# FishYuLi/BalancedGroupSoftmax

Measured on AMD Instinct MI355X. Metric: img/s fwd+bwd R50-FPN+BAGS 1333x800, 512 RoI (BASELINE metric: img/s/GPU fwd+bwd R50-FPN+BAGS 1333x800, 512 RoI; GroupSoftmax us/RoI), higher is better.
Workload: dtype f32 (conv/linear products on the bf16 MFMA from exact 3-way bf16 splits, fp32 accumulate: fp32-faithful)

## Files before the change

balancedgroupsoftmax_amd/backbone.py:

```python
import contextlib

import torch
import torch.nn as nn

from . import functional as BF
from .ops import OFFSET_PITCH, DeformConv
from .registry import BACKBONES, NECKS


def _trainable(*modules):
    return torch.is_grad_enabled() and any(
        p.requires_grad for m in modules if m is not None for p in m.parameters())


def _fold_conv_bn(conv, bn, pad_cin_to=None):
    w = conv.weight
    cbias = getattr(conv, 'bias', None)
    if w.is_cuda:
        ctx = contextlib.nullcontext() if _trainable(conv, bn) else torch.no_grad()
        with ctx:
            if bn is not None:
                return BF.fold_conv_bn(w, cbias, bn.weight, bn.bias, bn.running_mean,
                                       bn.running_var, bn.eps, cin_padded=pad_cin_to)
            return BF.fold_conv_bn(w, cbias, cin_padded=pad_cin_to)
# ... 148 lines not shown
        if self.groups > 1:
            out = BF.grouped_conv3x3_nhwc(out, f['c2'][0], f['c2'][1], self.groups, stride=self.stride,
                                          relu=True)
        else:
            out = BF.conv2d_nhwc(out, f['c2'][0], f['c2'][1], stride=self.stride, pad=1, relu=True)
        if fk is not None:
            fk.join()
        return BF.conv2d_nhwc(out, f['c3'][0], f['c3'][1], relu=True, residual=identity)

    def run(self, x, f, next_c1=None, h=None):
        if h is not None and (x.dtype == torch.bfloat16 or self.groups > 1 or self.with_dcn or
                              (torch.is_grad_enabled() and x.requires_grad)):
            raise RuntimeError('Bottleneck.run: a precomputed conv1 output is for the frozen fp32 block only')
        if x.dtype == torch.bfloat16:
            return self.run_bf16_storage(x, f)
        tagged = bool(getattr(x, '_bgs_consumers_mask', False))
        fuse = BF.fork_fusion_enabled() and torch.is_grad_enabled() and x.requires_grad
        if tagged and not fuse:
            raise RuntimeError("Bottleneck.run: x is a relu='consumers' block output but fork fusion is off")
        out_relu = 'consumers' if BF.fork_fusion_enabled() else True
        xin = x
        identity = x
        fk = None
        if 'ds' in f and not fuse and x.is_cuda and BF.shortcut_fork_enabled() and \
                not (torch.is_grad_enabled() and any(t.requires_grad for t in f['ds'] if t is not None)):
            with BF.forked(x.device) as fk:
                identity = BF.conv2d_nhwc(x, f['ds'][0], f['ds'][1], stride=self.stride)
        elif 'ds' in f:
            if fuse:
                identity, xin = BF.conv2d_autograd(x, f['ds'][0], f['ds'][1], stride=self.stride,
                                                   mask_input=tagged, passthrough=True)
            else:
                identity = BF.conv2d_autograd(x, f['ds'][0], f['ds'][1], stride=self.stride)
        first_pt = fuse and 'ds' not in f
        first_mask = tagged and 'ds' not in f
        if self.groups > 1 or self.with_dcn:
            out = BF.conv2d_autograd(xin, f['c1'][0], f['c1'][1], relu=True, mask_input=first_mask,
                                     passthrough=first_pt)
            if first_pt:
                out, identity = out
            if self.with_dcn:
                off = BF.conv2d_autograd(out, f['off'][0], f['off'][1], stride=self.stride, pad=1)
                out = BF.deform_conv3x3_nhwc(out, off, f['c2'][0], f['c2'][1], self.dcn_groups,
                                             stride=self.stride, relu=True)
            else:
                out = BF.grouped_conv3x3_nhwc(out, f['c2'][0], f['c2'][1], self.groups,
                                              stride=self.stride, relu=True)
            if fk is not None:
                fk.join()
            return BF.conv2d_autograd(out, f['c3'][0], f['c3'][1], relu=out_relu, residual=identity)
        if h is not None:
            out = h
        else:
            out = BF.conv2d_autograd(xin, f['c1'][0], f['c1'][1], relu='consumers', mask_input=first_mask,
                                     passthrough=first_pt)
            if first_pt:
                out, identity = out
        if not fuse and BF.fused_c3_eligible(out, f['c2'][0], f['c3'][0], self.stride, identity):
            if fk is not None:
                fk.join()
            if next_c1 is not None and BF.fused_c3_next_eligible(out, f['c2'][0], f['c3'][0], self.stride, identity,
                                                                 next_c1[0], next_c1[1]):
                return BF.conv3x3_c3_next_fused_nhwc(out, f['c2'][0], f['c2'][1], f['c3'][0], f['c3'][1], next_c1[0],
                                                     next_c1[1], residual=identity, relu3=True)
            return BF.conv3x3_c3_fused_nhwc(out, f['c2'][0], f['c2'][1], f['c3'][0], f['c3'][1], residual=identity,
                                            relu3=True)
        out = BF.conv2d_autograd(out, f['c2'][0], f['c2'][1], stride=self.stride, pad=1,
                                 relu='consumers', mask_input=True)
        if fk is not None:
            fk.join()
        return BF.conv2d_autograd(out, f['c3'][0], f['c3'][1], relu=out_relu, residual=identity,
                                  mask_input=True)


@BACKBONES.register_module
class ResNet(nn.Module):
    arch_settings = {50: (3, 4, 6, 3), 101: (3, 4, 23, 3), 152: (3, 8, 36, 3)}

    def __init__(self, depth, num_stages=4, strides=(1, 2, 2, 2), dilations=(1, 1, 1, 1),
                 out_indices=(0, 1, 2, 3), style='pytorch', frozen_stages=-1, conv_cfg=None,
# ... 217 lines not shown
```

balancedgroupsoftmax_amd/capi.py:

```python
import ctypes
import os

_PKG = os.path.dirname(os.path.abspath(__file__))

c_i64p = ctypes.c_void_p
c_f32p = ctypes.c_void_p
c_ptr = ctypes.c_void_p

BGS_OK = 0
BGS_MAX_BINS = 16


class BgsLibraryError(RuntimeError):
    pass


class BgsCallError(RuntimeError):
    def __init__(self, fn, code, text):
        super().__init__('%s failed with code %d: %s' % (fn, code, text))
        self.code = code


SIGNATURES = {
    'bgs_version': (ctypes.c_int, []),
# ... 56 lines not shown
                             + [c_f32p] * 4 + [c_ptr]),
    'bgs_conv2d_wgrad_bfx_workspace_bytes': (ctypes.c_size_t, [ctypes.c_int] * 9),
    'bgs_conv2d_wgrad_nhwc_f32_bfx': (ctypes.c_int, [c_f32p, c_f32p, c_f32p, c_f32p]
                                      + [ctypes.c_int] * 11 + [c_ptr, c_ptr]),
    'bgs_conv2d_wgrad_bfx_enable': (None, [ctypes.c_int]),
    'bgs_conv3x3_halo_nhwc_f32': (ctypes.c_int, [c_f32p, c_f32p, c_f32p, c_f32p] + [ctypes.c_int] * 6
                                  + [c_ptr]),
    'bgs_conv_bfx_weight_bytes': (ctypes.c_size_t, [ctypes.c_int, ctypes.c_int]),
    'bgs_conv_bfx_split_weights': (ctypes.c_int, [c_f32p, c_ptr, ctypes.c_int, ctypes.c_int, c_ptr]),
    'bgs_conv_dgrad_parity_enable': (None, [ctypes.c_int]),
    'bgs_conv_bfx_split_weights_dgrad': (ctypes.c_int, [c_f32p, c_ptr] + [ctypes.c_int] * 4 + [c_ptr]),
    'bgs_conv_bfx_workspace_bytes': (ctypes.c_size_t, [ctypes.c_longlong, ctypes.c_int, ctypes.c_int]),
    'bgs_conv2d_nhwc_f32_bfx_ws': (ctypes.c_int, [c_f32p, c_ptr, c_f32p, c_f32p, c_f32p]
                                   + [ctypes.c_int] * 12 + [c_ptr, ctypes.c_size_t, c_ptr]),
    'bgs_conv2d_dgrad_nhwc_f32_bfx_ws': (ctypes.c_int, [c_f32p, c_ptr, c_f32p, c_f32p, c_f32p]
                                         + [ctypes.c_int] * 11 + [c_ptr, ctypes.c_size_t, c_ptr]),
    'bgs_conv3x3_halo_bfx_workspace_bytes': (ctypes.c_size_t, [ctypes.c_int] * 5),
    'bgs_conv3x3_c3_fused_nhwc_f32_bfx': (ctypes.c_int, [c_f32p, c_ptr, c_f32p, c_ptr, c_f32p, c_f32p, c_f32p]
                                          + [ctypes.c_int] * 6 + [c_ptr]),
    'bgs_conv3x3_c3_next_fused_nhwc_f32_bfx': (ctypes.c_int,
                                               [c_f32p, c_ptr, c_f32p, c_ptr, c_f32p, c_f32p, c_f32p, c_ptr, c_f32p,
                                                c_f32p] + [ctypes.c_int] * 7 + [c_ptr]),
    'bgs_conv3x3_c3_next_eligible': (ctypes.c_int, [ctypes.c_int] * 6),
    'bgs_conv3x3_halo_nhwc_f32_bfx': (ctypes.c_int, [c_f32p, c_ptr, c_f32p, c_f32p]
                                      + [ctypes.c_int] * 7 + [c_ptr, ctypes.c_size_t, c_ptr]),
    'bgs_conv3x3_halo_nhwc_f32_bfx_ex': (ctypes.c_int, [c_f32p, c_ptr, c_f32p, c_f32p, c_f32p]
                                         + [ctypes.c_int] * 7 + [c_ptr, ctypes.c_size_t, c_ptr]),
    'bgs_conv3x3_planes_head_nhwc_f32_bfx': (ctypes.c_int, [c_f32p, c_ptr, c_f32p, c_ptr, c_f32p, c_f32p]
                                             + [ctypes.c_int] * 7 + [c_ptr]),
    'bgs_conv3x3_planes_head_eligible': (ctypes.c_int, [ctypes.c_int] * 6),
    'bgs_gs_loss_tuning': (None, [ctypes.c_int]),
    'bgs_gs_head_fold': (None, [ctypes.c_int]),
    'bgs_gs_loss_wavepriv_min_rows': (None, [ctypes.c_int]),
    'bgs_gs_merge_tuning': (None, [ctypes.c_int, ctypes.c_int]),
    'bgs_conv_bfx_wide_tuning': (None, [ctypes.c_int] * 3),
    'bgs_conv_bfx_wide_last_launch': (ctypes.c_int, []),
    'bgs_conv1x1_planes_enable': (None, [ctypes.c_int]),
    'bgs_conv1x1_planes_last_launch': (ctypes.c_int, []),
    'bgs_conv3x3_planes_enable': (None, [ctypes.c_int]),
    'bgs_conv3x3_planes_last_launch': (ctypes.c_int, []),
    'bgs_conv1x1_bres_enable': (None, [ctypes.c_int]),
    'bgs_conv1x1_bres_last_launch': (ctypes.c_int, []),
    'bgs_launch_census': (ctypes.c_int, [ctypes.c_int, ctypes.c_int]),
    'bgs_conv_bfx_tuning': (None, [ctypes.c_int] * 2),
    'bgs_conv_bfx_last_launch': (ctypes.c_int, [c_ptr, c_ptr]),
    'bgs_conv_tuning': (None, [ctypes.c_int] * 4),
# ... 235 lines not shown
```

balancedgroupsoftmax_amd/csrc/bottleneck_tail_planes.hip:

```cpp
#include <stdlib.h>

#include "conv_args.h"
#include "bfx_split.h"

using namespace bgs_conv;

namespace {

typedef __bf16 bf16x2 __attribute__((ext_vector_type(2)));
typedef __bf16 bf16x8 __attribute__((ext_vector_type(8)));
typedef unsigned u32x2 __attribute__((ext_vector_type(2)));
typedef unsigned u32x4 __attribute__((ext_vector_type(4)));

__device__ __forceinline__ unsigned pk_bf16(float a, float b) {
  const bf16x2 h = __builtin_convertvector(f32x2{a, b}, bf16x2);
  return __builtin_bit_cast(unsigned, h);
}

__device__ __forceinline__ void split3p(const f32x4 v, u32x2& hi, u32x2& mid, u32x2& lo) {
  hi = u32x2{pk_bf16(v[0], v[1]), pk_bf16(v[2], v[3])};
  const f32x4 r = {bfx_resid_lo(hi[0], v[0]), bfx_resid_hi(hi[0], v[1]), bfx_resid_lo(hi[1], v[2]),
                   bfx_resid_hi(hi[1], v[3])};
  mid = u32x2{pk_bf16(r[0], r[1]), pk_bf16(r[2], r[3])};
  const f32x4 r2 = {bfx_resid_lo(mid[0], r[0]), bfx_resid_hi(mid[0], r[1]), bfx_resid_lo(mid[1], r[2]),
                    bfx_resid_hi(mid[1], r[3])};
  lo = u32x2{pk_bf16(r2[0], r2[1]), pk_bf16(r2[2], r2[3])};
}

struct TailArgs {
  const float* x;
  const __bf16* ws2;
  const float* bias2;
  const __bf16* ws3;
  const float* bias3;
  const float* res;
  float* y;
  int N, H, W, relu3;
  int tiles_y, tiles_x, tiles, chunk;
};

struct TailNextArgs {
  TailArgs t;
  const __bf16* ws1n;
  const float* bias1n;
  float* h;
};
template <int NEXT> struct TailArgsOf { typedef TailNextArgs type; };
template <> struct TailArgsOf<0> { typedef TailArgs type; };
__device__ __forceinline__ const TailArgs& tail_base(const TailArgs& a) { return a; }
__device__ __forceinline__ const TailArgs& tail_base(const TailNextArgs& a) { return a.t; }

constexpr int kOob = 0x7f000000;

template <int NEXT>
__global__ __launch_bounds__(kThreads, 3) void bottleneck_tail_planes_kernel(typename TailArgsOf<NEXT>::type ga) {
  static_assert(NEXT == 0 || NEXT == 64 || NEXT == 128, "width of the next block's conv1");
  const TailArgs& g = tail_base(ga);
  constexpr int NS = 3, CM = 64, CO3 = 256, KC2 = 36, KC3 = 4;
  constexpr int PW = 10, PS = 12, PSLOTS = PW * PS;
  constexpr int AQ = PW * PW * 16, AQT = (AQ + kThreads - 1) / kThreads;
  constexpr int KS = PSLOTS * 32, PL = 4 * KS;
  constexpr int KCN = CO3 / 16, KCH = KCN / 2, KSN = 64 * 32 + 32, PLN = KCH * KSN;
  constexpr int LDS_BYTES = NEXT ? NS * PLN : NS * PL;
  static_assert(64 * (NEXT + 8) * 4 <= LDS_BYTES, "the h transpose tile overlays the planes");
  static_assert(NS * PL <= LDS_BYTES && 3 * LDS_BYTES <= 160 * 1024, "three workgroups per CU");
  constexpr int LD2 = CM + 4, S2_BYTES = 64 * LD2 * 4;
  constexpr int Y_OFF = 18 * 1024;
  constexpr int P3_CH = 64 * 32, P3_PL = KC3 * P3_CH;
  constexpr int LD4 = CO3 + 8;
  static_assert(S2_BYTES <= Y_OFF && Y_OFF + NS * P3_PL <= LDS_BYTES && 32 * LD4 * 4 <= LDS_BYTES, "overlays");
  __shared__ __attribute__((aligned(1024))) unsigned char lds[LDS_BYTES];

  const int tid = threadIdx.x, lane = tid & 63;
  const int wave = bgs::uniform(tid >> 6);
  const int wm = wave >> 1, wn = wave & 1;
  const int frow = lane & 31, fk = lane >> 5;
  const int vtile = (int)((blockIdx.x & 7) * g.chunk + (blockIdx.x >> 3));
  if (vtile >= g.tiles) return;
  const int per_img = g.tiles_y * g.tiles_x;
  const int n = vtile / per_img, trem = vtile - n * per_img;
  const int ty = trem / g.tiles_x, tx = trem - ty * g.tiles_x;
  const int h0 = ty * 8 - 1, w0 = tx * 8 - 1;

  const __amdgpu_buffer_rsrc_t x_rsrc = __builtin_amdgcn_make_buffer_rsrc(
      const_cast<float*>(g.x), 0, (int)((size_t)g.N * g.H * g.W * CM * 4), 0x00020000);
  f32x4 ra[AQT];
  int a_dst[AQT];
#pragma unroll
  for (int i = 0; i < AQT; ++i) {
    const int q = tid + kThreads * i;
    const bool use = q < AQ;
    const int pix = use ? q >> 4 : 0, kq = q & 15;
    const int ppy = pix / PW, ppx = pix - ppy * PW;
    const int hi = h0 + ppy, wi = w0 + ppx;
    const bool in = use && hi >= 0 && hi < g.H && wi >= 0 && wi < g.W;
    const int off = in ? (((n * g.H + hi) * g.W + wi) * CM + kq * 4) * 4 : kOob;
    ra[i] = __builtin_bit_cast(f32x4, __builtin_amdgcn_raw_buffer_load_b128(x_rsrc, off, 0, 0));
    const int quad = kq & 3;
    a_dst[i] = use ? (kq >> 2) * KS + (ppy * PS + ppx) * 32 + (((quad >> 1) ^ (ppy & 1)) << 4) + (quad & 1) * 8 : -1;
  }

  const __amdgpu_buffer_rsrc_t b2_rsrc = __builtin_amdgcn_make_buffer_rsrc(
      const_cast<__bf16*>(g.ws2), 0, NS * KC2 * CM * 32, 0x00020000);
  const int b2_lane = ((wn * 32 + frow) * 16 + fk * 8) * 2;
  auto load_b2 = [&](int kc, bf16x8 (&dst)[NS]) {
#pragma unroll
    for (int s = 0; s < NS; ++s)
      dst[s] = __builtin_bit_cast(bf16x8, __builtin_amdgcn_raw_buffer_load_b128(b2_rsrc, b2_lane, (s * KC2 + kc) * CM * 32, 0));
  };
  bf16x8 fbA[NS], fbB[NS];
  load_b2(0, fbA);

#pragma unroll
  for (int i = 0; i < AQT; ++i) {
    if (a_dst[i] < 0) continue;
    u32x2 hh, mm, ll;
    split3p(ra[i], hh, mm, ll);
    unsigned char* d = lds + a_dst[i];
    *reinterpret_cast<u32x2*>(d) = hh;
    *reinterpret_cast<u32x2*>(d + PL) = mm;
    *reinterpret_cast<u32x2*>(d + 2 * PL) = ll;
  }
  __syncthreads();

// ... 19 lines not shown
    bf16x8 fa[NS];
#pragma unroll
    for (int s = 0; s < NS; ++s)
      fa[s] = *reinterpret_cast<const bf16x8*>(lds + s * PL + c16 * KS + a_frag[dy & 1] + (dy * PS + dx) * 32);
#pragma unroll
    for (int tt = NS - 1; tt >= 0; --tt)
#pragma unroll
      for (int i = 0; i <= tt; ++i) acc2 = __builtin_amdgcn_mfma_f32_32x32x16_bf16(fa[i], fb[tt - i], acc2, 0, 0, 0);
    __builtin_amdgcn_sched_barrier(0);
  }

  const __amdgpu_buffer_rsrc_t b3_rsrc = __builtin_amdgcn_make_buffer_rsrc(
      const_cast<__bf16*>(g.ws3), 0, NS * KC3 * CO3 * 32, 0x00020000);
  const int b3_lane = ((wave * 64 + frow) * 16 + fk * 8) * 2;
  auto load_b3 = [&](int kc, bf16x8 (&dst)[NS][2]) {
#pragma unroll
    for (int s = 0; s < NS; ++s)
#pragma unroll
      for (int b = 0; b < 2; ++b)
        dst[s][b] = __builtin_bit_cast(bf16x8, __builtin_amdgcn_raw_buffer_load_b128(b3_rsrc, b3_lane, ((s * KC3 + kc) * CO3 + 32 * b) * 32, 0));
  };
  bf16x8 f3a[NS][2], f3b[NS][2];
  load_b3(0, f3a);

  __syncthreads();
  float* scratch = reinterpret_cast<float*>(lds);
#pragma unroll
  for (int r = 0; r < 16; ++r) {
    const int i = wm * 32 + (r & 3) + 8 * (r >> 2) + 4 * (lane >> 5);
    scratch[i * LD2 + wn * 32 + (lane & 31)] = acc2[r];
  }
  __syncthreads();
  {
    const int c4 = (tid & 15) * 4, r0 = tid >> 4;
    f32x4 bias2 = {0.f, 0.f, 0.f, 0.f};
    if (g.bias2) bias2 = *reinterpret_cast<const f32x4*>(g.bias2 + c4);
    const int kc2 = c4 >> 4, kq2 = (c4 & 15) >> 2;
#pragma unroll
    for (int ps = 0; ps < 4; ++ps) {
      const int i = r0 + ps * 16;
      f32x4 v = *reinterpret_cast<const f32x4*>(scratch + i * LD2 + c4);
      v += bias2;
#pragma unroll
      for (int t = 0; t < 4; ++t) v[t] = fmaxf(v[t], 0.f);
      u32x2 hh, mm, ll;
      split3p(v, hh, mm, ll);
// ... 3 lines not shown
      *reinterpret_cast<u32x2*>(d + 2 * P3_PL) = ll;
    }
  }
  __syncthreads();

  int a3_frag[2];
#pragma unroll
  for (int a = 0; a < 2; ++a) {
    const int m = a * 32 + frow;
    a3_frag[a] = Y_OFF + m * 32 + ((fk ^ ((m >> 3) & 1)) << 4);
  }
  f32x16 acc3[2][2];
#pragma unroll
  for (int a = 0; a < 2; ++a)
#pragma unroll
    for (int b = 0; b < 2; ++b)
#pragma unroll
      for (int r = 0; r < 16; ++r) acc3[a][b][r] = 0.f;
#pragma unroll
  for (int kc = 0; kc < KC3; ++kc) {
    if (kc + 1 < KC3) {
      if (kc & 1) load_b3(kc + 1, f3a);
      else load_b3(kc + 1, f3b);
    }
    __builtin_amdgcn_sched_barrier(0);
    const bf16x8 (&fb3)[NS][2] = (kc & 1) ? f3b : f3a;
    bf16x8 fa3[NS][2];
#pragma unroll
    for (int s = 0; s < NS; ++s)
#pragma unroll
      for (int a = 0; a < 2; ++a) fa3[s][a] = *reinterpret_cast<const bf16x8*>(lds + a3_frag[a] + kc * P3_CH + s * P3_PL);
#pragma unroll
    for (int tt = NS - 1; tt >= 0; --tt)
#pragma unroll
      for (int i = 0; i <= tt; ++i)
#pragma unroll
        for (int a = 0; a < 2; ++a)
#pragma unroll
          for (int b = 0; b < 2; ++b)
            acc3[a][b] = __builtin_amdgcn_mfma_f32_32x32x16_bf16(fa3[i][a], fb3[tt - i][b], acc3[a][b], 0, 0, 0);
    __builtin_amdgcn_sched_barrier(0);
  }
  __syncthreads();

  const int e4 = (tid & 63) * 4, er0 = tid >> 6;
  f32x4 bias3 = {0.f, 0.f, 0.f, 0.f};
  if (g.bias3) bias3 = *reinterpret_cast<const f32x4*>(g.bias3 + e4);
  const int out_bytes = (int)((size_t)g.N * g.H * g.W * CO3 * 4);
  const __amdgpu_buffer_rsrc_t res_rsrc = __builtin_amdgcn_make_buffer_rsrc(
      const_cast<float*>(g.res ? g.res : g.x), 0, g.res ? out_bytes : 0, 0x00020000);
  const __amdgpu_buffer_rsrc_t y_rsrc = __builtin_amdgcn_make_buffer_rsrc(g.y, 0, out_bytes, 0x00020000);
  f32x4 vn[NEXT ? 2 : 1][NEXT ? 8 : 1];
#pragma unroll
  for (int a = 0; a < 2; ++a) {
    f32x4 rs[8];
#pragma unroll
    for (int ps = 0; ps < 8; ++ps) {
      const int m = a * 32 + er0 + ps * 4;
      const int ho = min(ty * 8 + (m >> 3), g.H - 1), wo = min(tx * 8 + (m & 7), g.W - 1);
      rs[ps] = __builtin_bit_cast(f32x4, __builtin_amdgcn_raw_buffer_load_b128(res_rsrc, (((n * g.H + ho) * g.W + wo) * CO3 + e4) * 4, 0, 0));
    }
#pragma unroll
    for (int b = 0; b < 2; ++b)
#pragma unroll
      for (int r = 0; r < 16; ++r) {
        const int i = (r & 3) + 8 * (r >> 2) + 4 * (lane >> 5);
        scratch[i * LD4 + wave * 64 + b * 32 + (lane & 31)] = acc3[a][b][r];
      }
    __syncthreads();
#pragma unroll
    for (int ps = 0; ps < 8; ++ps) {
      const int i = er0 + ps * 4;
      const int m = a * 32 + i;
      const int ho = ty * 8 + (m >> 3), wo = tx * 8 + (m & 7);
      f32x4 v = *reinterpret_cast<const f32x4*>(scratch + i * LD4 + e4);
      v += bias3;
      v += rs[ps];
      if (g.relu3) {
#pragma unroll
        for (int t = 0; t < 4; ++t) v[t] = fmaxf(v[t], 0.f);
      }
      if (ho < g.H && wo < g.W)
        __builtin_amdgcn_raw_buffer_store_b128(__builtin_bit_cast(u32x4, v), y_rsrc, (((n * g.H + ho) * g.W + wo) * CO3 + e4) * 4, 0, 0);
      if constexpr (NEXT > 0) vn[a][ps] = v;
    }
    __syncthreads();
  }

  if constexpr (NEXT > 0) {
    constexpr int LDH = NEXT + 8, NA = NEXT == 128 ? 2 : 1;
    const int a0 = NEXT == 128 ? 0 : (wave >> 1);
    const int tn = NEXT == 128 ? wave : (wave & 1);
    const __amdgpu_buffer_rsrc_t bn_rsrc = __builtin_amdgcn_make_buffer_rsrc(
        const_cast<__bf16*>(ga.ws1n), 0, NS * KCN * NEXT * 32, 0x00020000);
    const int bn_lane = ((tn * 32 + frow) * 16 + fk * 8) * 2;
    auto load_bn = [&](int kc, bf16x8 (&dst)[NS]) {
#pragma unroll
      for (int s = 0; s < NS; ++s)
        dst[s] = __builtin_bit_cast(bf16x8, __builtin_amdgcn_raw_buffer_load_b128(bn_rsrc, bn_lane, (s * KCN + kc) * NEXT * 32, 0));
    };
    bf16x8 fn[3][NS];
    load_bn(0, fn[0]);
    load_bn(1, fn[1]);
    f32x4 vs[2][8];
#pragma unroll
    for (int ps = 0; ps < 8; ++ps) {
      const u32x4 lo = __builtin_bit_cast(u32x4, vn[0][ps]), hi = __builtin_bit_cast(u32x4, vn[1][ps]);
      u32x4 slo, shi;
#pragma unroll
      for (int t = 0; t < 4; ++t) {
        const unsigned a0 = lo[t], a1 = hi[t];
        const auto sw = __builtin_amdgcn_permlane32_swap(a0, a1, false, false);
        slo[t] = sw[0];
        shi[t] = sw[1];
      }
      vs[0][ps] = __builtin_bit_cast(f32x4, slo);
      vs[1][ps] = __builtin_bit_cast(f32x4, shi);
// ... 36 lines not shown
          for (int a = 0; a < NA; ++a) fan[s][a] = *reinterpret_cast<const bf16x8*>(lds + s * PLN + k8 * KSN + an_frag[a]);
#pragma unroll
        for (int tt = NS - 1; tt >= 0; --tt)
#pragma unroll
          for (int i = 0; i <= tt; ++i)
#pragma unroll
            for (int a = 0; a < NA; ++a)
              accn[a] = __builtin_amdgcn_mfma_f32_32x32x16_bf16(fan[i][a], fbn[tt - i], accn[a], 0, 0, 0);
        __builtin_amdgcn_sched_barrier(0);
      }
      __syncthreads();
    }
#pragma unroll
    for (int a = 0; a < NA; ++a)
#pragma unroll
      for (int r = 0; r < 16; ++r) {
        const int i = (a0 + a) * 32 + (r & 3) + 8 * (r >> 2) + 4 * (lane >> 5);
        scratch[i * LDH + tn * 32 + (lane & 31)] = accn[a][r];
      }
    __syncthreads();
    constexpr int TPRN = NEXT / 4, RPPN = kThreads / TPRN, EPN = 64 / RPPN;
    const int n4 = (tid % TPRN) * 4, nr0 = tid / TPRN;
    f32x4 biasn = {0.f, 0.f, 0.f, 0.f};
    if (ga.bias1n) biasn = *reinterpret_cast<const f32x4*>(ga.bias1n + n4);
    const __amdgpu_buffer_rsrc_t h_rsrc =
        __builtin_amdgcn_make_buffer_rsrc(ga.h, 0, (int)((size_t)g.N * g.H * g.W * NEXT * 4), 0x00020000);
#pragma unroll
    for (int ps = 0; ps < EPN; ++ps) {
      const int m = nr0 + ps * RPPN;
      const int ho = ty * 8 + (m >> 3), wo = tx * 8 + (m & 7);
      f32x4 v = *reinterpret_cast<const f32x4*>(scratch + m * LDH + n4);
      v += biasn;
#pragma unroll
      for (int t = 0; t < 4; ++t) v[t] = fmaxf(v[t], 0.f);
      if (ho < g.H && wo < g.W)
        __builtin_amdgcn_raw_buffer_store_b128(__builtin_bit_cast(u32x4, v), h_rsrc, (((n * g.H + ho) * g.W + wo) * NEXT + n4) * 4, 0, 0);
    }
  }
}

}

int bgs_internal_bottleneck_tail_planes(const float* x, const void* w2split, const float* bias2, const void* w3split,
                                        const float* bias3, const float* residual, float* y, int N, int H, int W,
                                        int relu3, hipStream_t st) {
  const long long lim = kOob;
  if ((long long)N * H * W * 256 * 4 >= lim) return -1;
  TailArgs g;
  g.x = x;
// ... 31 lines not shown
  TailArgs& g = a.t;
  g.x = x;
  g.ws2 = reinterpret_cast<const __bf16*>(w2split);
  g.bias2 = bias2;
  g.ws3 = reinterpret_cast<const __bf16*>(w3split);
  g.bias3 = bias3;
  g.res = residual;
  g.y = y;
  g.N = N; g.H = H; g.W = W; g.relu3 = relu3;
  g.tiles_y = (H + 7) / 8;
  g.tiles_x = (W + 7) / 8;
  g.tiles = N * g.tiles_y * g.tiles_x;
  g.chunk = (g.tiles + 7) / 8;
  a.ws1n = reinterpret_cast<const __bf16*>(w1n_split);
  a.bias1n = bias1n;
  a.h = h;
  const dim3 grid((unsigned)(8 * g.chunk)), block(kThreads);
  if (Cnext == 64) hipLaunchKernelGGL(bottleneck_tail_planes_kernel<64>, grid, block, 0, (hipStream_t)stream, a);
  else hipLaunchKernelGGL(bottleneck_tail_planes_kernel<128>, grid, block, 0, (hipStream_t)stream, a);
  bgs_internal_census_bump(BGS_CENSUS_FUSED_C3);
  bgs_internal_census_bump(BGS_CENSUS_FUSED_C3_NEXT);
  return hipGetLastError() == hipSuccess ? BGS_OK : BGS_ERR_LAUNCH;
}
```

balancedgroupsoftmax_amd/functional.py:

```python
import ctypes
import itertools
import os

import torch

from . import capi

_WS = {}


def _workspace(nbytes, device):
    key = (device.index, capi.raw_stream(device))
    buf = _WS.get(key)
    if buf is None or buf.numel() < nbytes:
        buf = torch.empty(max(int(nbytes), 1 << 20), dtype=torch.uint8, device=device)
        _WS[key] = buf
    return buf


def reset_workspaces():
    _WS.clear()


_SIDE = {}
# ... 736 lines not shown
    lib.bgs_conv_bfx_tuning(int(tile), int(splitk))
    lib.bgs_conv3x3_halo_bfx_tuning(int(halo_splits), int(halo_variant) | ((int(halo_geom) + 1) << 16) |
                                    (int(halo_flags) << 20) | ((int(halo_wide) + 1) << 24))


def set_halo_wide(mode):
    return capi.load().bgs_conv3x3_halo_bfx_wide(int(mode))


def conv_bfx_last_launch():
    import ctypes
    lib = capi.load()
    a, c, d, e, f, g = (ctypes.c_int() for _ in range(6))
    lib.bgs_conv_bfx_last_launch(ctypes.byref(a), ctypes.byref(c))
    lib.bgs_conv3x3_halo_bfx_last_launch(ctypes.byref(d), ctypes.byref(e))
    lib.bgs_conv3x3_halo_bfx_last_wide(ctypes.byref(f), ctypes.byref(g))
    return dict(tile=a.value & ~0x400, ring_stages=3 if a.value & 0x400 else 4, splits=c.value,
                halo_nb=d.value & 0xff, halo_variant=(d.value >> 8) & 0xff, halo_geom=d.value >> 16,
                halo_splits=e.value, halo_wide_units=f.value, halo_tail_units=g.value)


CENSUS = dict(bf16_ring8=0, grouped_lds=1, halo_bfx4=2, dma_ring64=3, gs_head_fused=4, conv1x1_bres=5,
              wgrad_bfx=6, roi_bwd_gather=7, bf16s=8, grouped_bf16s=9, bfx_wide=10, gs_scale_grad=11, halo_wide=12, stem_fused=13, fused_c3=14,
              planes_3x3=15, planes_1x1=16, planes_3x3_head=17, fused_c3_next=18)


def launch_census(reset=False):
    lib = capi.load()
    out = {k: lib.bgs_launch_census(v, 0) for k, v in CENSUS.items()}
    if reset:
        lib.bgs_launch_census(0, 1)
    return out


def conv_tuning(tile=0, bk=0, splitk=0, noswizzle=0):
    capi.load().bgs_conv_tuning(int(tile), int(bk), int(splitk), int(noswizzle))


def conv_last_launch():
    import ctypes
    a, b, c, d = (ctypes.c_int() for _ in range(4))
    capi.load().bgs_conv_last_launch(ctypes.byref(a), ctypes.byref(b), ctypes.byref(c), ctypes.byref(d))
    return dict(tile=a.value, bk=b.value, up=c.value, splits=d.value)


def _use_halo_bfx(M, Cout):
    env = os.environ.get('BGS_CONV_HALO')
# ... 69 lines not shown


def conv3x3_c3_next_fused_nhwc(x, w2_krsc, bias2, w3_krsc, bias3, w1n_krsc, bias1n, residual=None, relu3=True):
    _require_cuda(x, w2_krsc, bias2, w3_krsc, bias3, w1n_krsc, bias1n, residual)
    lib = capi.load()
    assert x.dtype == torch.float32 and x.is_contiguous() and x.dim() == 4
    N, H, W, Cmid = x.shape
    Cout3, Cnext = w3_krsc.shape[0], w1n_krsc.shape[0]
    assert tuple(w2_krsc.shape) == (Cmid, 3, 3, Cmid) and tuple(w3_krsc.shape) == (Cout3, 1, 1, Cmid)
    assert tuple(w1n_krsc.shape) == (Cnext, 1, 1, Cout3) and w1n_krsc.is_contiguous()
    if residual is not None:
        assert tuple(residual.shape) == (N, H, W, Cout3) and residual.is_contiguous() and residual.dtype == torch.float32
    y = torch.empty((N, H, W, Cout3), dtype=torch.float32, device=x.device)
    h = torch.empty((N, H, W, Cnext), dtype=torch.float32, device=x.device)
    w2s = bfx_split_weights(w2_krsc.view(Cmid, 9 * Cmid), cache=True)
    w3s = bfx_split_weights(w3_krsc.view(Cout3, Cmid), cache=True)
    w1s = bfx_split_weights(w1n_krsc.view(Cnext, Cout3), cache=True)
    rc = lib.bgs_conv3x3_c3_next_fused_nhwc_f32_bfx(capi.ptr(x), capi.ptr(w2s), capi.ptr(bias2), capi.ptr(w3s),
                                                    capi.ptr(bias3), capi.ptr(residual), capi.ptr(y), capi.ptr(w1s),
                                                    capi.ptr(bias1n), capi.ptr(h), N, H, W, Cmid, Cout3,
                                                    int(bool(relu3)), Cnext, capi.current_stream(x.device))
    capi.check('bgs_conv3x3_c3_next_fused_nhwc_f32_bfx', rc)
    return y, h


def rpn_head_fusion_eligible(x, w_conv, w_head):
    if os.environ.get('BGS_RPN_HEAD_FUSION', '1') == '0' or _CONV_MATH[0] != 'bf16x6':
        return False
    if not x.is_cuda or x.dtype != torch.float32 or x.dim() != 4 or w_conv.dim() != 4 or w_head.dim() != 4:
        return False
    N, H, W, Cin = x.shape
    if tuple(w_conv.shape[1:]) != (3, 3, Cin) or tuple(w_head.shape[1:]) != (1, 1, w_conv.shape[0]):
        return False
    if not _use_halo_bfx(N * H * W, w_conv.shape[0]):
        return False
    return bool(capi.load().bgs_conv3x3_planes_head_eligible(N, H, W, Cin, w_conv.shape[0], w_head.shape[0]))


def conv3x3_head_fused_nhwc(x, w_krsc, bias, hw_krsc, hbias, relu=True):
    _require_cuda(x, w_krsc, bias, hw_krsc, hbias)
    lib = capi.load()
    assert x.dtype == torch.float32 and x.is_contiguous() and x.dim() == 4
    N, H, W, Cin = x.shape
    Cout, Ch = w_krsc.shape[0], hw_krsc.shape[0]
    assert tuple(w_krsc.shape) == (Cout, 3, 3, Cin) and tuple(hw_krsc.shape) == (Ch, 1, 1, Cout)
    assert w_krsc.is_contiguous() and hw_krsc.is_contiguous()
# ... 1856 lines not shown
```

include/bgs.h:

```cpp
#ifndef BGS_H_
#define BGS_H_

#include <stddef.h>
#include <stdint.h>

#ifdef __cplusplus
extern "C" {
#endif

#define BGS_OK 0
#define BGS_ERR_INVALID_ARG 1
#define BGS_ERR_UNSUPPORTED 2
#define BGS_ERR_LAUNCH 3

#define BGS_MAX_BINS 16

typedef void* bgs_stream_t;

int bgs_version(void);
const char* bgs_error_string(int code);



int bgs_gs_prepare(const int64_t* labels, const int64_t* label2binlabel,
// ... 104 lines not shown
int bgs_conv2d_dgrad_nhwc_f32_bfx_ws(const float* dy, const void* wt_split, const float* residual,
                                     const float* mask, float* dx, int N, int H, int W, int Cin,
                                     int Cout, int R, int S, int stride, int pad,
                                     int residual_mode, int planes, void* workspace,
                                     size_t workspace_bytes, bgs_stream_t stream);
size_t bgs_conv3x3_halo_bfx_workspace_bytes(int N, int H, int W, int Cin, int Cout);
int bgs_conv3x3_halo_nhwc_f32_bfx(const float* x, const void* wsplit, const float* bias, float* y,
                                  int N, int H, int W, int Cin, int Cout, int relu, int planes,
                                  void* workspace, size_t workspace_bytes, bgs_stream_t stream);
int bgs_conv3x3_halo_nhwc_f32_bfx_ex(const float* x, const void* wsplit, const float* bias,
                                     const float* mask, float* y, int N, int H, int W, int Cin,
                                     int Cout, int relu, int planes, void* workspace,
                                     size_t workspace_bytes, bgs_stream_t stream);
int bgs_conv3x3_c3_fused_nhwc_f32_bfx(const float* x, const void* w2split, const float* bias2,
                                      const void* w3split, const float* bias3, const float* residual,
                                      float* y, int N, int H, int W, int Cmid, int Cout3, int relu3,
                                      bgs_stream_t stream);
int bgs_conv3x3_c3_next_fused_nhwc_f32_bfx(const float* x, const void* w2split, const float* bias2,
                                           const void* w3split, const float* bias3, const float* residual,
                                           float* y, const void* w1n_split, const float* bias1n, float* h,
                                           int N, int H, int W, int Cmid, int Cout3, int relu3, int Cnext,
                                           bgs_stream_t stream);
int bgs_conv3x3_c3_next_eligible(int N, int H, int W, int Cmid, int Cout3, int Cnext);
int bgs_conv3x3_planes_head_nhwc_f32_bfx(const float* x, const void* wsplit, const float* bias,
                                         const void* hsplit, const float* hbias, float* y, int N, int H,
                                         int W, int Cin, int Cout, int relu, int Chead, bgs_stream_t stream);
int bgs_conv3x3_planes_head_eligible(int N, int H, int W, int Cin, int Cout, int Chead);


int bgs_grouped_conv3x3_nhwc_f32(const float* x, const float* w, const float* bias, float* y,
                                 int N, int H, int W, int C, int groups, int stride, int relu,
                                 bgs_stream_t stream);

int bgs_grouped_conv3x3_nhwc_bf16ops(const float* x, const float* w, const float* bias, float* y,
                                     int N, int H, int W, int C, int groups, int stride, int relu,
                                     bgs_stream_t stream);

int bgs_conv2d_nhwc_bf16s(const void* x, const void* w_hi, const float* bias, const void* residual,
                          int residual_mode, int residual_bf16, void* y, int y_bf16, int N, int H, int W,
                          int Cin, int Cout, int R, int S, int stride, int pad, int relu,
                          bgs_stream_t stream);
int bgs_grouped_conv3x3_nhwc_bf16s(const void* x, const float* w, const float* bias, void* y, int N, int H,
                                   int W, int C, int groups, int stride, int relu, bgs_stream_t stream);
int bgs_maxpool3x3s2_nhwc_f32_to_bf16(const float* x, void* y, int N, int H, int W, int C,
                                      bgs_stream_t stream);

// ... 258 lines not shown
```

include/bgs_tuning.h:

```cpp
#ifndef BGS_TUNING_H_
#define BGS_TUNING_H_

#include "bgs.h"

#ifdef __cplusplus
extern "C" {
#endif

int bgs_selftest_wave_reduce(const float* in, float* out, bgs_stream_t stream);
int bgs_selftest_mfma_peak(int blocks, int iters, float* out, bgs_stream_t stream);
int bgs_selftest_mfma_peak_bf16(int blocks, int iters, int random_operands, float* out, bgs_stream_t stream);

#define BGS_CENSUS_BF16_RING8 0
#define BGS_CENSUS_GROUPED_LDS 1
#define BGS_CENSUS_HALO_BFX4 2
#define BGS_CENSUS_DMA_RING64 3
#define BGS_CENSUS_GS_HEAD_FUSED 4
#define BGS_CENSUS_CONV1X1_BRES 5
#define BGS_CENSUS_WGRAD_BFX 6
#define BGS_CENSUS_ROI_BWD_GATHER 7
#define BGS_CENSUS_BF16S 8
#define BGS_CENSUS_GROUPED_BF16S 9
#define BGS_CENSUS_BFX_WIDE 10
#define BGS_CENSUS_GS_SCALE_GRAD 11
#define BGS_CENSUS_HALO_WIDE 12
#define BGS_CENSUS_STEM_FUSED 13
#define BGS_CENSUS_FUSED_C3 14
#define BGS_CENSUS_PLANES_3X3 15
#define BGS_CENSUS_PLANES_1X1 16
#define BGS_CENSUS_PLANES_3X3_HEAD 17
#define BGS_CENSUS_FUSED_C3_NEXT 18
#define BGS_CENSUS_FAMILIES 20
int bgs_launch_census(int family, int reset);

void bgs_gs_head_debug_timestamps(unsigned long long* buf);
void bgs_gs_head_tuning(int rows_per_workgroup);
void bgs_gs_head_fold(int on);
void bgs_gs_head_variant(int variant);
int bgs_gs_head_variant_used(int N);

void bgs_conv_tuning(int tile, int bk, int splitk, int noswizzle);
int bgs_conv_last_launch(int* tile, int* bk, int* up, int* splits);
void bgs_conv_bfx_tuning(int tile, int splitk);
int bgs_conv_bfx_last_launch(int* tile, int* splits);
void bgs_conv3x3_halo_bfx_tuning(int splits, int variant);
int bgs_conv3x3_halo_bfx_last_launch(int* nb, int* splits);
int bgs_conv3x3_halo_bfx_last_wide(int* wide_units, int* tail_units);
int bgs_conv3x3_halo_bfx_wide(int mode);
void bgs_conv1x1_bres_enable(int on);
int bgs_conv1x1_bres_last_launch(void);
void bgs_conv_dgrad_parity_enable(int on);
void bgs_conv2d_wgrad_bfx_enable(int on);
void bgs_conv_bf16s_tuning(int variant);

// ... 16 lines not shown
```

Baseline: 428.3.

## Fuse layer1.0 projection shortcut conv into the bottleneck tail kernel

Adds a shortcut variant of the fused conv3x3+conv1x1 tail kernel. It also computes the stride-1 64->256 projection shortcut from the block input inside the epilogue, using 3-way bf16 splits on MFMA, and adds it to the c3 output. This removes a separate downsample conv launch and its 256-channel identity write and read-back. The cost is extra LDS, more registers and serial MFMA work in the epilogue. It applies only to frozen, no-grad blocks like layer1.0.

```diff
diff --git a/balancedgroupsoftmax_amd/backbone.py b/balancedgroupsoftmax_amd/backbone.py
--- a/balancedgroupsoftmax_amd/backbone.py
+++ b/balancedgroupsoftmax_amd/backbone.py
@@ -194,7 +194,14 @@
         xin = x
         identity = x
         fk = None
-        if 'ds' in f and not fuse and x.is_cuda and BF.shortcut_fork_enabled() and \
+        sc_tail = ('ds' in f and not fuse and self.groups == 1 and not self.with_dcn and x.is_cuda and
+                   not (torch.is_grad_enabled() and any(t.requires_grad for k in ('c1', 'c2', 'c3', 'ds') for t in f[k]
+                                                        if t is not None)) and
+                   BF.fused_c3_shortcut_eligible(x, tuple(x.shape[:3]) + (f['c1'][0].shape[0],), f['c2'][0], f['c3'][0],
+                                                 self.stride, f['ds'][0], f['ds'][1], self.stride))
+        if sc_tail:
+            identity = None
+        elif 'ds' in f and not fuse and x.is_cuda and BF.shortcut_fork_enabled() and \
                 not (torch.is_grad_enabled() and any(t.requires_grad for t in f['ds'] if t is not None)):
             with BF.forked(x.device) as fk:
                 identity = BF.conv2d_nhwc(x, f['ds'][0], f['ds'][1], stride=self.stride)
@@ -228,6 +235,13 @@
                                      passthrough=first_pt)
             if first_pt:
                 out, identity = out
+        if sc_tail:
+            if BF.fused_c3_eligible(out, f['c2'][0], f['c3'][0], self.stride, None):
+                nc = next_c1 if next_c1 is not None and next_c1[0].shape[0] == 64 and BF.fused_c3_next_eligible(
+                    out, f['c2'][0], f['c3'][0], self.stride, None, next_c1[0], next_c1[1]) else (None, None)
+                return BF.conv3x3_c3_sc_fused_nhwc(out, f['c2'][0], f['c2'][1], f['c3'][0], f['c3'][1], x, f['ds'][0],
+                                                   f['ds'][1], nc[0], nc[1], relu3=True)
+            identity = BF.conv2d_nhwc(x, f['ds'][0], f['ds'][1], stride=self.stride)
         if not fuse and BF.fused_c3_eligible(out, f['c2'][0], f['c3'][0], self.stride, identity):
             if fk is not None:
                 fk.join()
diff --git a/balancedgroupsoftmax_amd/capi.py b/balancedgroupsoftmax_amd/capi.py
--- a/balancedgroupsoftmax_amd/capi.py
+++ b/balancedgroupsoftmax_amd/capi.py
@@ -102,6 +102,10 @@
                                                [c_f32p, c_ptr, c_f32p, c_ptr, c_f32p, c_f32p, c_f32p, c_ptr, c_f32p,
                                                 c_f32p] + [ctypes.c_int] * 7 + [c_ptr]),
     'bgs_conv3x3_c3_next_eligible': (ctypes.c_int, [ctypes.c_int] * 6),
+    'bgs_conv3x3_c3_sc_fused_nhwc_f32_bfx': (ctypes.c_int,
+                                             [c_f32p, c_ptr, c_f32p, c_ptr, c_f32p, c_f32p, c_ptr, c_f32p, c_f32p, c_ptr,
+                                              c_f32p, c_f32p] + [ctypes.c_int] * 8 + [c_ptr]),
+    'bgs_conv3x3_c3_sc_eligible': (ctypes.c_int, [ctypes.c_int] * 7),
     'bgs_conv3x3_halo_nhwc_f32_bfx': (ctypes.c_int, [c_f32p, c_ptr, c_f32p, c_f32p]
                                       + [ctypes.c_int] * 7 + [c_ptr, ctypes.c_size_t, c_ptr]),
     'bgs_conv3x3_halo_nhwc_f32_bfx_ex': (ctypes.c_int, [c_f32p, c_ptr, c_f32p, c_f32p, c_f32p]
diff --git a/balancedgroupsoftmax_amd/csrc/bottleneck_tail_planes.hip b/balancedgroupsoftmax_amd/csrc/bottleneck_tail_planes.hip
--- a/balancedgroupsoftmax_amd/csrc/bottleneck_tail_planes.hip
+++ b/balancedgroupsoftmax_amd/csrc/bottleneck_tail_planes.hip
@@ -45,29 +45,66 @@
   const float* bias1n;
   float* h;
 };
-template <int NEXT> struct TailArgsOf { typedef TailNextArgs type; };
-template <> struct TailArgsOf<0> { typedef TailArgs type; };
+template <class A> struct TailScArgs {
+  A a;
+  const float* x0;
+  const __bf16* wssc;
+  const float* bias_sc;
+};
+template <int NEXT, bool SC = false> struct TailArgsOf { typedef TailNextArgs type; };
+template <> struct TailArgsOf<0, false> { typedef TailArgs type; };
+template <int NEXT> struct TailArgsOf<NEXT, true> { typedef TailScArgs<typename TailArgsOf<NEXT>::type> type; };
 __device__ __forceinline__ const TailArgs& tail_base(const TailArgs& a) { return a; }
 __device__ __forceinline__ const TailArgs& tail_base(const TailNextArgs& a) { return a.t; }
+template <class A> __device__ __forceinline__ const TailArgs& tail_base(const TailScArgs<A>& a) { return tail_base(a.a); }
+template <class A> __device__ __forceinline__ const A& tail_inner(const A& a) { return a; }
+template <class A> __device__ __forceinline__ const A& tail_inner(const TailScArgs<A>& a) { return a.a; }
 
 constexpr int kOob = 0x7f000000;
 
-template <int NEXT>
-__global__ __launch_bounds__(kThreads, 3) void bottleneck_tail_planes_kernel(typename TailArgsOf<NEXT>::type ga) {
+__device__ __forceinline__ void load_x0_half(const float* x0, const TailArgs& g, int n, int ty, int tx, int tid, int a,
+                                             f32x4& q0, f32x4& q1) {
+  const __amdgpu_buffer_rsrc_t x0_rsrc = __builtin_amdgcn_make_buffer_rsrc(
+      const_cast<float*>(x0), 0, (int)((size_t)g.N * g.H * g.W * 64 * 4), 0x00020000);
+  f32x4 q[2];
+#pragma unroll
+  for (int j = 0; j < 2; ++j) {
+    const int m = a * 32 + (tid >> 4) + 16 * j;
+    const int ho = ty * 8 + (m >> 3), wo = tx * 8 + (m & 7);
+    const int off = ho < g.H && wo < g.W ? (((n * g.H + ho) * g.W + wo) * 64 + (tid & 15) * 4) * 4 : kOob;
+    q[j] = __builtin_bit_cast(f32x4, __builtin_amdgcn_raw_buffer_load_b128(x0_rsrc, off, 0, 0));
+  }
+  q0 = q[0];
+  q1 = q[1];
+}
+
+__device__ __forceinline__ void load_sc_filter(const __bf16* wssc, int lane_off, int t, bf16x8 (&dst)[3]) {
+  const __amdgpu_buffer_rsrc_t bs_rsrc = __builtin_amdgcn_make_buffer_rsrc(const_cast<__bf16*>(wssc), 0, 3 * 4 * 256 * 32, 0x00020000);
+#pragma unroll
+  for (int s = 0; s < 3; ++s)
+    dst[s] = __builtin_bit_cast(bf16x8, __builtin_amdgcn_raw_buffer_load_b128(bs_rsrc, lane_off, ((s * 4 + (t & 3)) * 256 + 32 * (t >> 2)) * 32, 0));
+}
+
+template <int NEXT, bool SC = false>
+__global__ __launch_bounds__(kThreads, 3) void bottleneck_tail_planes_kernel(typename TailArgsOf<NEXT, SC>::type ga) {
   static_assert(NEXT == 0 || NEXT == 64 || NEXT == 128, "width of the next block's conv1");
+  static_assert(!SC || NEXT != 128, "a block with a stride-1 projection shortcut (layer1.0) is never in front of a 128-wide conv1");
   const TailArgs& g = tail_base(ga);
+  const auto& gn = tail_inner(ga);
   constexpr int NS = 3, CM = 64, CO3 = 256, KC2 = 36, KC3 = 4;
   constexpr int PW = 10, PS = 12, PSLOTS = PW * PS;
   constexpr int AQ = PW * PW * 16, AQT = (AQ + kThreads - 1) / kThreads;
   constexpr int KS = PSLOTS * 32, PL = 4 * KS;
   constexpr int KCN = CO3 / 16, KCH = KCN / 2, KSN = 64 * 32 + 32, PLN = KCH * KSN;
-  constexpr int LDS_BYTES = NEXT ? NS * PLN : NS * PL;
+  constexpr int LD4 = CO3 + 8;
+  constexpr int SC_OFF = 32 * LD4 * 4, KSC = 32 * 32 + 32, PLSC = KC3 * KSC;
+  constexpr int LDS_BASE = NEXT ? NS * PLN : NS * PL;
+  constexpr int LDS_BYTES = SC && SC_OFF + NS * PLSC > LDS_BASE ? SC_OFF + NS * PLSC : LDS_BASE;
   static_assert(64 * (NEXT + 8) * 4 <= LDS_BYTES, "the h transpose tile overlays the planes");
   static_assert(NS * PL <= LDS_BYTES && 3 * LDS_BYTES <= 160 * 1024, "three workgroups per CU");
   constexpr int LD2 = CM + 4, S2_BYTES = 64 * LD2 * 4;
   constexpr int Y_OFF = 18 * 1024;
   constexpr int P3_CH = 64 * 32, P3_PL = KC3 * P3_CH;
-  constexpr int LD4 = CO3 + 8;
   static_assert(S2_BYTES <= Y_OFF && Y_OFF + NS * P3_PL <= LDS_BYTES && 32 * LD4 * 4 <= LDS_BYTES, "overlays");
   __shared__ __attribute__((aligned(1024))) unsigned char lds[LDS_BYTES];
 
@@ -100,6 +137,9 @@
     a_dst[i] = use ? (kq >> 2) * KS + (ppy * PS + ppx) * 32 + (((quad >> 1) ^ (ppy & 1)) << 4) + (quad & 1) * 8 : -1;
   }
 
+  f32x4 rx[SC ? 4 : 1];
+  if constexpr (SC) load_x0_half(ga.x0, g, n, ty, tx, tid, 0, rx[0], rx[1]);
+
   const __amdgpu_buffer_rsrc_t b2_rsrc = __builtin_amdgcn_make_buffer_rsrc(
       const_cast<__bf16*>(g.ws2), 0, NS * KC2 * CM * 32, 0x00020000);
   const int b2_lane = ((wn * 32 + frow) * 16 + fk * 8) * 2;
@@ -165,6 +205,7 @@
   };
   bf16x8 f3a[NS][2], f3b[NS][2];
   load_b3(0, f3a);
+  bf16x8 fsa[NS], fsb[NS];
 
   __syncthreads();
   float* scratch = reinterpret_cast<float*>(lds);
@@ -214,6 +255,12 @@
     if (kc + 1 < KC3) {
       if (kc & 1) load_b3(kc + 1, f3a);
       else load_b3(kc + 1, f3b);
+    }
+    if constexpr (SC) {
+      if (kc == KC3 - 1) {
+        load_sc_filter(ga.wssc, b3_lane, 0, fsa);
+        load_x0_half(ga.x0, g, n, ty, tx, tid, 1, rx[2], rx[3]);
+      }
     }
     __builtin_amdgcn_sched_barrier(0);
     const bf16x8 (&fb3)[NS][2] = (kc & 1) ? f3b : f3a;
@@ -243,6 +290,83 @@
       const_cast<float*>(g.res ? g.res : g.x), 0, g.res ? out_bytes : 0, 0x00020000);
   const __amdgpu_buffer_rsrc_t y_rsrc = __builtin_amdgcn_make_buffer_rsrc(g.y, 0, out_bytes, 0x00020000);
   f32x4 vn[NEXT ? 2 : 1][NEXT ? 8 : 1];
+  if constexpr (SC) {
+    const int kcw = (tid & 15) >> 2, kqw = tid & 3;
+    auto write_planes = [&](int a) {
+#pragma unroll
+      for (int j = 0; j < 2; ++j) {
+        const int i = (tid >> 4) + 16 * j;
+        u32x2 hh, mm, ll;
+        split3p(rx[2 * a + j], hh, mm, ll);
+        unsigned char* d = lds + SC_OFF + kcw * KSC + i * 32 + (((kqw >> 1) ^ ((i >> 3) & 1)) << 4) + (kqw & 1) * 8;
+        *reinterpret_cast<u32x2*>(d) = hh;
+        *reinterpret_cast<u32x2*>(d + PLSC) = mm;
+        *reinterpret_cast<u32x2*>(d + 2 * PLSC) = ll;
+      }
+    };
+    const int as_frag = SC_OFF + frow * 32 + ((fk ^ ((frow >> 3) & 1)) << 4);
+    float b3v[2] = {0.f, 0.f}, bsv[2] = {0.f, 0.f};
+#pragma unroll
+    for (int b = 0; b < 2; ++b) {
+      if (g.bias3) b3v[b] = g.bias3[wave * 64 + b * 32 + (lane & 31)];
+      if (ga.bias_sc) bsv[b] = ga.bias_sc[wave * 64 + b * 32 + (lane & 31)];
+    }
+    write_planes(0);
+#pragma unroll
+    for (int a = 0; a < 2; ++a) {
+      __syncthreads();
+#pragma unroll
+      for (int b = 0; b < 2; ++b) {
+        f32x16 accs;
+#pragma unroll
+        for (int r = 0; r < 16; ++r) accs[r] = 0.f;
+#pragma unroll
+        for (int kc = 0; kc < KC3; ++kc) {
+          const int t = b * KC3 + kc;
+          if (t + 1 < 2 * KC3) {
+            if (t & 1) load_sc_filter(ga.wssc, b3_lane, t + 1, fsa);
+            else load_sc_filter(ga.wssc, b3_lane, t + 1, fsb);
+          }
+          __builtin_amdgcn_sched_barrier(0);
+          const bf16x8 (&fbs)[NS] = (t & 1) ? fsb : fsa;
+          bf16x8 fas[NS];
+#pragma unroll
+          for (int s = 0; s < NS; ++s) fas[s] = *reinterpret_cast<const bf16x8*>(lds + as_frag + kc * KSC + s * PLSC);
+#pragma unroll
+          for (int tt = NS - 1; tt >= 0; --tt)
+#pragma unroll
+            for (int i = 0; i <= tt; ++i) accs = __builtin_amdgcn_mfma_f32_32x32x16_bf16(fas[i], fbs[tt - i], accs, 0, 0, 0);
+          __builtin_amdgcn_sched_barrier(0);
+        }
+#pragma unroll
+        for (int r = 0; r < 16; ++r) {
+          const int i = (r & 3) + 8 * (r >> 2) + 4 * (lane >> 5);
+          const float rsc = accs[r] + bsv[b];
+          scratch[i * LD4 + wave * 64 + b * 32 + (lane & 31)] = (acc3[a][b][r] + b3v[b]) + rsc;
+        }
+      }
+      __syncthreads();
+      if (a == 0) {
+        load_sc_filter(ga.wssc, b3_lane, 0, fsa);
+        write_planes(1);
+      }
+#pragma unroll
+      for (int ps = 0; ps < 8; ++ps) {
+        const int i = er0 + ps * 4;
+        const int m = a * 32 + i;
+        const int ho = ty * 8 + (m >> 3), wo = tx * 8 + (m & 7);
+        f32x4 v = *reinterpret_cast<const f32x4*>(scratch + i * LD4 + e4);
+        if (g.relu3) {
+#pragma unroll
+          for (int t = 0; t < 4; ++t) v[t] = fmaxf(v[t], 0.f);
+        }
+        if (ho < g.H && wo < g.W)
+          __builtin_amdgcn_raw_buffer_store_b128(__builtin_bit_cast(u32x4, v), y_rsrc, (((n * g.H + ho) * g.W + wo) * CO3 + e4) * 4, 0, 0);
+        if constexpr (NEXT > 0) vn[a][ps] = v;
+      }
+    }
+    if constexpr (NEXT > 0) __syncthreads();
+  } else {
 #pragma unroll
   for (int a = 0; a < 2; ++a) {
     f32x4 rs[8];
@@ -278,13 +402,14 @@
     }
     __syncthreads();
   }
+  }
 
   if constexpr (NEXT > 0) {
     constexpr int LDH = NEXT + 8, NA = NEXT == 128 ? 2 : 1;
     const int a0 = NEXT == 128 ? 0 : (wave >> 1);
     const int tn = NEXT == 128 ? wave : (wave & 1);
     const __amdgpu_buffer_rsrc_t bn_rsrc = __builtin_amdgcn_make_buffer_rsrc(
-        const_cast<__bf16*>(ga.ws1n), 0, NS * KCN * NEXT * 32, 0x00020000);
+        const_cast<__bf16*>(gn.ws1n), 0, NS * KCN * NEXT * 32, 0x00020000);
     const int bn_lane = ((tn * 32 + frow) * 16 + fk * 8) * 2;
     auto load_bn = [&](int kc, bf16x8 (&dst)[NS]) {
 #pragma unroll
@@ -367,9 +492,9 @@
     constexpr int TPRN = NEXT / 4, RPPN = kThreads / TPRN, EPN = 64 / RPPN;
     const int n4 = (tid % TPRN) * 4, nr0 = tid / TPRN;
     f32x4 biasn = {0.f, 0.f, 0.f, 0.f};
-    if (ga.bias1n) biasn = *reinterpret_cast<const f32x4*>(ga.bias1n + n4);
+    if (gn.bias1n) biasn = *reinterpret_cast<const f32x4*>(gn.bias1n + n4);
     const __amdgpu_buffer_rsrc_t h_rsrc =
-        __builtin_amdgcn_make_buffer_rsrc(ga.h, 0, (int)((size_t)g.N * g.H * g.W * NEXT * 4), 0x00020000);
+        __builtin_amdgcn_make_buffer_rsrc(gn.h, 0, (int)((size_t)g.N * g.H * g.W * NEXT * 4), 0x00020000);
 #pragma unroll
     for (int ps = 0; ps < EPN; ++ps) {
       const int m = nr0 + ps * RPPN;
@@ -447,3 +572,61 @@
   bgs_internal_census_bump(BGS_CENSUS_FUSED_C3_NEXT);
   return hipGetLastError() == hipSuccess ? BGS_OK : BGS_ERR_LAUNCH;
 }
+
+extern "C" int bgs_conv3x3_c3_sc_eligible(int N, int H, int W, int Cin0, int Cmid, int Cout3, int Cnext) {
+  if (N <= 0 || H <= 0 || W <= 0 || Cin0 != 64 || Cmid != 64 || Cout3 != 256 || (Cnext != 0 && Cnext != 64)) return 0;
+  const long long lim = kOob / (256 * 4);
+  const long long nh = (long long)N * H;
+  if (nh >= lim) return 0;
+  return nh * W < lim ? 1 : 0;
+}
+
+extern "C" int bgs_conv3x3_c3_sc_fused_nhwc_f32_bfx(const float* x, const void* w2split, const float* bias2,
+                                                    const void* w3split, const float* bias3, const float* x0,
+                                                    const void* wsc_split, const float* bias_sc, float* y,
+                                                    const void* w1n_split, const float* bias1n, float* h, int N, int H,
+                                                    int W, int Cin0, int Cmid, int Cout3, int relu3, int Cnext,
+                                                    bgs_stream_t stream) {
+  if (N <= 0 || H <= 0 || W <= 0 || !x || !w2split || !w3split || !x0 || !wsc_split || !y) return BGS_ERR_INVALID_ARG;
+  if (Cnext != 0 && (!w1n_split || !h)) return BGS_ERR_INVALID_ARG;
+  if (!bgs_conv3x3_c3_sc_eligible(N, H, W, Cin0, Cmid, Cout3, Cnext)) return BGS_ERR_UNSUPPORTED;
+  if (((uintptr_t)x | (uintptr_t)w2split | (uintptr_t)w3split | (uintptr_t)y | (uintptr_t)x0 | (uintptr_t)wsc_split |
+       (uintptr_t)bias2 | (uintptr_t)bias3 | (uintptr_t)bias_sc) % 16 != 0)
+    return BGS_ERR_UNSUPPORTED;
+  if (Cnext != 0 && ((uintptr_t)w1n_split | (uintptr_t)bias1n | (uintptr_t)h) % 16 != 0) return BGS_ERR_UNSUPPORTED;
+  TailScArgs<TailNextArgs> a;
+  TailArgs& g = a.a.t;
+  g.x = x;
+  g.ws2 = reinterpret_cast<const __bf16*>(w2split);
+  g.bias2 = bias2;
+  g.ws3 = reinterpret_cast<const __bf16*>(w3split);
+  g.bias3 = bias3;
+  g.res = nullptr;
+  g.y = y;
+  g.N = N; g.H = H; g.W = W; g.relu3 = relu3;
+  g.tiles_y = (H + 7) / 8;
+  g.tiles_x = (W + 7) / 8;
+  g.tiles = N * g.tiles_y * g.tiles_x;
+  g.chunk = (g.tiles + 7) / 8;
+  a.a.ws1n = reinterpret_cast<const __bf16*>(w1n_split);
+  a.a.bias1n = bias1n;
+  a.a.h = h;
+  a.x0 = x0;
+  a.wssc = reinterpret_cast<const __bf16*>(wsc_split);
+  a.bias_sc = bias_sc;
+  const dim3 grid((unsigned)(8 * g.chunk)), block(kThreads);
+  if (Cnext == 64) {
+    hipLaunchKernelGGL((bottleneck_tail_planes_kernel<64, true>), grid, block, 0, (hipStream_t)stream, a);
+    bgs_internal_census_bump(BGS_CENSUS_FUSED_C3_NEXT);
+  } else {
+    TailScArgs<TailArgs> a0;
+    a0.a = g;
+    a0.x0 = a.x0;
+    a0.wssc = a.wssc;
+    a0.bias_sc = a.bias_sc;
+    hipLaunchKernelGGL((bottleneck_tail_planes_kernel<0, true>), grid, block, 0, (hipStream_t)stream, a0);
+  }
+  bgs_internal_census_bump(BGS_CENSUS_FUSED_C3);
+  bgs_internal_census_bump(BGS_CENSUS_FUSED_C3_SHORTCUT);
+  return hipGetLastError() == hipSuccess ? BGS_OK : BGS_ERR_LAUNCH;
+}
diff --git a/balancedgroupsoftmax_amd/functional.py b/balancedgroupsoftmax_amd/functional.py
--- a/balancedgroupsoftmax_amd/functional.py
+++ b/balancedgroupsoftmax_amd/functional.py
@@ -782,7 +782,7 @@
 
 CENSUS = dict(bf16_ring8=0, grouped_lds=1, halo_bfx4=2, dma_ring64=3, gs_head_fused=4, conv1x1_bres=5,
               wgrad_bfx=6, roi_bwd_gather=7, bf16s=8, grouped_bf16s=9, bfx_wide=10, gs_scale_grad=11, halo_wide=12, stem_fused=13, fused_c3=14,
-              planes_3x3=15, planes_1x1=16, planes_3x3_head=17, fused_c3_next=18)
+              planes_3x3=15, planes_1x1=16, planes_3x3_head=17, fused_c3_next=18, fused_c3_shortcut=19)
 
 
 def launch_census(reset=False):
@@ -898,6 +898,54 @@
                                                     int(bool(relu3)), Cnext, capi.current_stream(x.device))
     capi.check('bgs_conv3x3_c3_next_fused_nhwc_f32_bfx', rc)
     return y, h
+
+
+def fused_c3_shortcut_eligible(x0, h1_shape, w2, w3, stride, w_sc, b_sc=None, stride_sc=1):
+    if os.environ.get('BGS_TAIL_SHORTCUT', '1') == '0' or os.environ.get('BGS_FUSED_C3_PLANES', '1') == '0':
+        return False
+    if w_sc is None or w_sc.dim() != 4 or stride_sc != 1 or stride != 1:
+        return False
+    if tuple(w_sc.shape) != (256, 1, 1, 64) or w_sc.dtype != torch.float32 or not w_sc.is_contiguous():
+        return False
+    if x0.dim() != 4 or x0.shape[3] != 64 or x0.dtype != torch.float32 or not x0.is_cuda or not x0.is_contiguous():
+        return False
+    if tuple(h1_shape) != (x0.shape[0], x0.shape[1], x0.shape[2], 64):
+        return False
+    if torch.is_grad_enabled() and (x0.requires_grad or w_sc.requires_grad or (b_sc is not None and b_sc.requires_grad)):
+        return False
+    if not fused_c3_eligible(x0, w2, w3, stride, None):
+        return False
+    N, H, W, _ = x0.shape
+    return bool(capi.load().bgs_conv3x3_c3_sc_eligible(N, H, W, 64, 64, 256, 0))
+
+
+def conv3x3_c3_sc_fused_nhwc(x, w2_krsc, bias2, w3_krsc, bias3, x0, w_sc_krsc, bias_sc, w1n_krsc=None, bias1n=None,
+                             relu3=True):
+    _require_cuda(x, w2_krsc, bias2, w3_krsc, bias3, x0, w_sc_krsc, bias_sc, w1n_krsc, bias1n)
+    lib = capi.load()
+    assert x.dtype == torch.float32 and x.is_contiguous() and x.dim() == 4
+    N, H, W, Cmid = x.shape
+    Cout3, Cin0 = w3_krsc.shape[0], x0.shape[3]
+    Cnext = 0 if w1n_krsc is None else w1n_krsc.shape[0]
+    assert tuple(w2_krsc.shape) == (Cmid, 3, 3, Cmid) and tuple(w3_krsc.shape) == (Cout3, 1, 1, Cmid)
+    assert tuple(x0.shape) == (N, H, W, Cin0) and x0.is_contiguous() and x0.dtype == torch.float32
+    assert tuple(w_sc_krsc.shape) == (Cout3, 1, 1, Cin0) and w_sc_krsc.is_contiguous()
+    y = torch.empty((N, H, W, Cout3), dtype=torch.float32, device=x.device)
+    w2s = bfx_split_weights(w2_krsc.view(Cmid, 9 * Cmid), cache=True)
+    w3s = bfx_split_weights(w3_krsc.view(Cout3, Cmid), cache=True)
+    wss = bfx_split_weights(w_sc_krsc.view(Cout3, Cin0), cache=True)
+    h = w1s = None
+    if Cnext:
+        assert tuple(w1n_krsc.shape) == (Cnext, 1, 1, Cout3) and w1n_krsc.is_contiguous()
+        h = torch.empty((N, H, W, Cnext), dtype=torch.float32, device=x.device)
+        w1s = bfx_split_weights(w1n_krsc.view(Cnext, Cout3), cache=True)
+    rc = lib.bgs_conv3x3_c3_sc_fused_nhwc_f32_bfx(capi.ptr(x), capi.ptr(w2s), capi.ptr(bias2), capi.ptr(w3s),
+                                                  capi.ptr(bias3), capi.ptr(x0), capi.ptr(wss), capi.ptr(bias_sc),
+                                                  capi.ptr(y), capi.ptr(w1s), capi.ptr(bias1n if Cnext else None),
+                                                  capi.ptr(h), N, H, W, Cin0, Cmid, Cout3, int(bool(relu3)), Cnext,
+                                                  capi.current_stream(x.device))
+    capi.check('bgs_conv3x3_c3_sc_fused_nhwc_f32_bfx', rc)
+    return (y, h) if Cnext else y
 
 
 def rpn_head_fusion_eligible(x, w_conv, w_head):
diff --git a/include/bgs.h b/include/bgs.h
--- a/include/bgs.h
+++ b/include/bgs.h
@@ -150,6 +150,12 @@
                                            int N, int H, int W, int Cmid, int Cout3, int relu3, int Cnext,
                                            bgs_stream_t stream);
 int bgs_conv3x3_c3_next_eligible(int N, int H, int W, int Cmid, int Cout3, int Cnext);
+int bgs_conv3x3_c3_sc_fused_nhwc_f32_bfx(const float* x, const void* w2split, const float* bias2,
+                                         const void* w3split, const float* bias3, const float* x0,
+                                         const void* wsc_split, const float* bias_sc, float* y,
+                                         const void* w1n_split, const float* bias1n, float* h, int N, int H, int W,
+                                         int Cin0, int Cmid, int Cout3, int relu3, int Cnext, bgs_stream_t stream);
+int bgs_conv3x3_c3_sc_eligible(int N, int H, int W, int Cin0, int Cmid, int Cout3, int Cnext);
 int bgs_conv3x3_planes_head_nhwc_f32_bfx(const float* x, const void* wsplit, const float* bias,
                                          const void* hsplit, const float* hbias, float* y, int N, int H,
                                          int W, int Cin, int Cout, int relu, int Chead, bgs_stream_t stream);
diff --git a/include/bgs_tuning.h b/include/bgs_tuning.h
--- a/include/bgs_tuning.h
+++ b/include/bgs_tuning.h
@@ -30,6 +30,7 @@
 #define BGS_CENSUS_PLANES_1X1 16
 #define BGS_CENSUS_PLANES_3X3_HEAD 17
 #define BGS_CENSUS_FUSED_C3_NEXT 18
+#define BGS_CENSUS_FUSED_C3_SHORTCUT 19
 #define BGS_CENSUS_FAMILIES 20
 int bgs_launch_census(int family, int reset);
 
```

Result: faster. 434.6, median of 6 (+1.5%).
